# FIT-2023-SLAM-indoor/slam-indoor-code

Hardware: AMD Instinct MI355X
Metric: frames/sec (extract+match+BA) @1080p 10k kpts, 1/2/4/8 GPU; final reproj RMSE (higher is better)
Workload: dtype u8/i8 (int8 MFMA distances, f32 SIFT)

## Files before the change

### slam-indoor-code_amd/csrc/api.cpp

```cpp
#include <algorithm>
#include <cstdlib>
#include <chrono>
#include <cfloat>
#include <cmath>
#include <cstring>
#include <vector>

#include "slamhip_internal.h"

namespace slamhip {

hipError_t DevBuf::ensure(size_t n)
{
    if (n <= bytes && p) return hipSuccess;
    if (p) { (void)hipFree(p); p = nullptr; bytes = 0; }
    size_t want = n < 256 ? 256 : n;
    want = (want + 4095) & ~(size_t)4095;
    hipError_t e = hipMalloc(&p, want);
    if (e == hipSuccess) bytes = want;
    return e;
}

void DevBuf::release()
{
// ... 337 lines not shown
{
    int n = 0;
    if (hipGetDeviceCount(&n) != hipSuccess || device < 0 || device >= n) return nullptr;
    if (hipSetDevice(device) != hipSuccess) return nullptr;
    slam_ctx* c = new slam_ctx();
    c->device = device;
    int least = 0, greatest = 0;
    hipError_t e;
    if (priority > 0 && hipDeviceGetStreamPriorityRange(&least, &greatest) == hipSuccess)
        e = hipStreamCreateWithPriority(&c->stream, hipStreamNonBlocking, greatest);
    else
        e = hipStreamCreateWithFlags(&c->stream, hipStreamNonBlocking);
    if (e != hipSuccess) {
        delete c;
        return nullptr;
    }
    hipDeviceProp_t prop;
    if (hipGetDeviceProperties(&prop, device) == hipSuccess && prop.multiProcessorCount > 0)
        c->cu_count = prop.multiProcessorCount;
    init_consts(c);
    return c;
}

void slam_destroy(slam_ctx* c)
{
    if (!c) return;
    (void)hipSetDevice(c->device);
    (void)hipStreamSynchronize(c->stream);
    DevBuf* bufs[] = {&c->gray, &c->scores, &c->masks, &c->band_cnt, &c->band_pref, &c->frame_info, &c->ftmp,
                      &c->grad, &c->orbblur, &c->kps, &c->kp_frame, &c->desc_u8, &c->desc_f32,
                      &c->desc_norm, &c->desc_exp, &c->query_norm, &c->knn_part, &c->match_rec, &c->match_flag,
                      &c->match_cnt, &c->match_out, &c->frames_in, &c->qbuf, &c->tbuf, &c->misc, &c->ba_obs,
                      &c->ba_par, &c->ba_jac, &c->ba_red, &c->ba_S, &c->ba_aux, &c->sd_pyr, &c->sd_cand,
                      &c->sd_kps, &c->sd_kpc, &c->sift_tab, &c->sift_band_buf, &c->sift_cols_buf, &c->sift_cols_park, &c->sift_colw_buf, &c->sift_split, &c->sift_split_cnt, &c->geom, &c->cluster, &c->delaunay};
    for (DevBuf* b : bufs) b->release();
    if (c->h_up) (void)hipHostFree(c->h_up);
    if (c->ev_up) (void)hipEventDestroy(c->ev_up);
    if (c->h_rb) (void)hipHostFree(c->h_rb);
    if (c->h_win) (void)hipHostFree(c->h_win);
    if (c->ev_win) (void)hipEventDestroy(c->ev_win);
    if (c->ev_rdev) (void)hipEventDestroy(c->ev_rdev);
    if (c->ev_order) (void)hipEventDestroy(c->ev_order);
    for (hipEvent_t e : c->ev_stage)
        if (e) (void)hipEventDestroy(e);
    if (c->h_async) (void)hipHostFree(c->h_async);
    for (auto& f : c->prof)
        for (hipEvent_t e : f.ev) (void)hipEventDestroy(e);
    if (c->ev_sync) (void)hipEventDestroy(c->ev_sync);
    (void)hipStreamDestroy(c->stream);
    delete c;
}

const char* slam_last_error(const slam_ctx* c) { return c ? c->err.c_str() : "no context"; }

int slam_synchronize(slam_ctx* c)
{
    if (!c) return SLAM_E_INVALID_ARG;
    return stream_sync(c, c->stream);
}

int slam_matcher_type(int use_sift_bf, int use_sift_flann, int use_orb)
{
    if (use_sift_bf) return SLAM_SIFT_BF;
    if (use_sift_flann) return SLAM_SIFT_FLANN;
    if (use_orb) return SLAM_ORB_BF;
    return SLAM_E_BAD_MATCHER;
}
// ... 1025 lines not shown
```

### slam-indoor-code_amd/csrc/fast.hip

```cpp
#include "slamhip_internal.h"

namespace slamhip {

namespace {

constexpr int TW = kFastTileW, TH = 4 * kFastTileH;
constexpr int HALO = 4;
constexpr int LW = TW + 2 * HALO;
constexpr int LH = TH + 2 * HALO;
constexpr int SW = TW + 2, SH = TH + 2;
constexpr int SWP = LW;
constexpr int NG = SWP / 4;
static_assert(NG * 4 >= SW + 2, "the last group of a row is past the score columns");
constexpr int kBandsPerTile = TH / kFastTileH;
constexpr int kFastThreads = 256, kFastWaves = kFastThreads / 64;
static_assert(TH % kFastTileH == 0 && kFastWaves % kBandsPerTile == 0 && TH % kFastWaves == 0,
              "whole bands per tile, whole waves per band");
static_assert(TH * 16 % kFastThreads == 0, "whole gray store passes");

struct DetectParams {
    const uint8_t* img;
    size_t frame_stride, row_stride;
    int channels, w, h, thr, border;
    int ntx, nbands;
// ... 322 lines not shown
            int mx = max(max(sc[r][c], sc[r][c + 1]), sc[r][c + 2]);
            mx = max(mx, max(sc[r + 1][c], sc[r + 1][c + 2]));
            mx = max(mx, max(max(sc[r + 2][c], sc[r + 2][c + 1]), sc[r + 2][c + 2]));
            keep = s > mx;
        }
        const int gx = tx * TW + c;
        keep = keep && gx < p.w;
        const bool keepf = keep && gx >= bx && gx < p.w - bx && gy >= bx && gy < p.h - bx;
        kraw |= (uint32_t)keep << (c - 16 * qd);
        kfil |= (uint32_t)keepf << (c - 16 * qd);
        if (keepf) p.scores[(size_t)f * p.w * p.h + (size_t)gy * p.w + gx] = (uint8_t)s;
    }
    uint32_t lo32 = qd == 0 ? kfil : (qd == 1 ? kfil << 16 : 0u);
    uint32_t hi32 = qd == 2 ? kfil : (qd == 3 ? kfil << 16 : 0u);
    lo32 |= __shfl_xor(lo32, 1, 64);
    hi32 |= __shfl_xor(hi32, 1, 64);
    lo32 |= __shfl_xor(lo32, 2, 64);
    hi32 |= __shfl_xor(hi32, 2, 64);
    if (qd == 0 && gy < p.h) p.masks[((size_t)f * p.h + gy) * p.ntx + tx] = ((uint64_t)hi32 << 32) | lo32;
    int craw = __popc(kraw), cfil = __popc(kfil);
#pragma unroll
    for (int o = 32; o > 0; o >>= 1) {
        craw += __shfl_xor(craw, o, 64);
        cfil += __shfl_xor(cfil, o, 64);
    }
    const int band = ty * kBandsPerTile + (tid >> 6);
    if (lane == 0 && band < p.nbands) {
        int* bc = p.band_cnt + ((size_t)f * p.nbands + band) * 2;
        if (craw) atomicAdd(&bc[0], craw);
        if (cfil) atomicAdd(&bc[1], cfil);
    }
}

__global__ __launch_bounds__(1024) void fast_finalize(const int* band_cnt, int nframes, int nbands,
                                                      int* band_pref, int4* frame_info, int* total, int cap)
{
    __shared__ int cnt[1024];
    __shared__ int raw[1024];
    const int lane = threadIdx.x & 63, wave = threadIdx.x >> 6;
    for (int base = 0; base < nframes; base += 1024) {
        for (int fl = wave; fl < 1024 && base + fl < nframes; fl += 16) {
            const int f = base + fl;
            int run = 0, rsum = 0;
            for (int b0 = 0; b0 < nbands; b0 += 64) {
                const int b = b0 + lane;
                int c = 0, r = 0;
                if (b < nbands) {
                    c = band_cnt[((size_t)f * nbands + b) * 2 + 1];
                    r = band_cnt[((size_t)f * nbands + b) * 2 + 0];
                }
                int incl = c;
#pragma unroll
                for (int o = 1; o < 64; o <<= 1) {
                    const int v = __shfl_up(incl, o, 64);
                    if (lane >= o) incl += v;
                }
                if (b < nbands) band_pref[(size_t)f * nbands + b] = run + incl - c;
                run += __shfl(incl, 63, 64);
#pragma unroll
                for (int o = 32; o > 0; o >>= 1) r += __shfl_xor(r, o, 64);
                rsum += r;
            }
            if (lane == 0) { cnt[fl] = run; raw[fl] = rsum; }
        }
        __syncthreads();
        if (threadIdx.x == 0) {
            int off = base == 0 ? 0 : *total;
            for (int i = 0; i < 1024 && base + i < nframes; i++) {
                frame_info[base + i] = make_int4(off, min(cnt[i], max(cap - off, 0)), raw[i], 0);
                off += cnt[i];
            }
            *total = off;
        }
        __syncthreads();
// ... 106 lines not shown
    static const int dbg = [] { return diag_env_int("SLAMHIP_FAST_DBG"); }();
    p.dbg = dbg;
    p.gray = c->gray.as<uint8_t>(); p.masks = c->masks.as<uint64_t>(); p.scores = c->scores.as<uint8_t>();
    p.band_cnt = c->band_cnt.as<int>();
    c->batch.ntx = ntx;
    c->batch.nbands = nbands;
    dim3 grid(ntx, nty, nframes);
    prof_begin(c, 0, s);
    if (type == SLAM_FAST_TYPE_9_16) {
        if (nonmax) hipLaunchKernelGGL((fast_detect<1, 16>), grid, dim3(kFastThreads), 0, s, p);
        else hipLaunchKernelGGL((fast_detect<0, 16>), grid, dim3(kFastThreads), 0, s, p);
    } else if (type == SLAM_FAST_TYPE_7_12) {
        if (nonmax) hipLaunchKernelGGL((fast_detect<1, 12>), grid, dim3(kFastThreads), 0, s, p);
        else hipLaunchKernelGGL((fast_detect<0, 12>), grid, dim3(kFastThreads), 0, s, p);
    } else {
        if (nonmax) hipLaunchKernelGGL((fast_detect<1, 8>), grid, dim3(kFastThreads), 0, s, p);
        else hipLaunchKernelGGL((fast_detect<0, 8>), grid, dim3(kFastThreads), 0, s, p);
    }
    prof_end(c, 0, s);
    return hipGetLastError();
}

hipError_t launch_fast_emit(slam_ctx* c, hipStream_t s, int nframes, int w, int h, int cap)
{
    const int ntx = c->batch.ntx, nbands = c->batch.nbands;
    if (ntx * kFastTileH > 1024) return hipErrorInvalidValue;
    c->fast_gen++;
    hipError_t e;
    if ((e = c->band_pref.ensure((size_t)nframes * nbands * sizeof(int))) != hipSuccess) return e;
    if ((e = c->frame_info.ensure((size_t)nframes * sizeof(int4))) != hipSuccess) return e;
    if ((e = c->misc.ensure(256)) != hipSuccess) return e;
    if ((e = c->kps.ensure((size_t)cap * sizeof(slam_keypoint))) != hipSuccess) return e;
    if ((e = c->kp_frame.ensure((size_t)cap * sizeof(int))) != hipSuccess) return e;
    hipLaunchKernelGGL(fast_finalize, dim3(1), dim3(1024), 0, s, c->band_cnt.as<int>(), nframes, nbands,
                       c->band_pref.as<int>(), c->frame_info.as<int4>(), c->misc.as<int>(), cap);
    EmitParams p;
    p.masks = c->masks.as<uint64_t>(); p.scores = c->scores.as<uint8_t>();
    p.band_pref = c->band_pref.as<int>(); p.frame_info = c->frame_info.as<int4>();
    p.w = w; p.h = h; p.ntx = ntx; p.nbands = nbands; p.cap = cap;
    p.kps = c->kps.as<slam_keypoint>(); p.kp_frame = c->kp_frame.as<int>();
    hipLaunchKernelGGL(fast_emit, dim3(nbands, nframes), dim3(1024), 0, s, p);
    return hipGetLastError();
}

}
```

### slam-indoor-code_amd/csrc/knn.hip

```cpp
#include <cfloat>
#include <climits>
#include <cstdlib>

#include <type_traits>

#include "slamhip_internal.h"

namespace slamhip {

namespace {

typedef int v4i __attribute__((ext_vector_type(4)));
typedef int v16i __attribute__((ext_vector_type(16)));
typedef int v8i __attribute__((ext_vector_type(8)));
typedef float v16f __attribute__((ext_vector_type(16)));

enum { MODE_L2 = 0, MODE_HAM = 1, MODE_SQRT = 2, MODE_L2P = 3, MODE_HAMP = 4, MODE_L1P = 5 };

struct KnnParams {
    const uint8_t* q;
    const int* qnorm;
    int nq;
    const uint8_t* t;
    const int* tnorm;
// ... 686 lines not shown
        if (p.mode == MODE_L2) {
            const int qn = p.qnorm[q];
            if (x0 >= 0) d0 = cr_sqrtf((float)(qn + e0));
            if (x1 >= 0) d1 = cr_sqrtf((float)(qn + e1));
        } else if (p.mode == MODE_HAM) {
            if (x0 >= 0) d0 = (float)((256 + e0) / 2);
            if (x1 >= 0) d1 = (float)((256 + e1) / 2);
        } else if (p.mode == MODE_L2P) {
            const int qn = p.qnorm[q];
            if (x0 >= 0) d0 = cr_sqrtf((float)(qn + e0 - (1 << 21)));
            if (x1 >= 0) d1 = cr_sqrtf((float)(qn + e1 - (1 << 21)));
        } else if (p.mode == MODE_HAMP) {
            if (x0 >= 0) d0 = (float)(e0 / 2);
            if (x1 >= 0) d1 = (float)(e1 / 2);
        } else if (p.mode == MODE_L1P) {
            if (x0 >= 0) d0 = (float)e0;
            if (x1 >= 0) d1 = (float)e1;
        } else {
            if (x0 >= 0) d0 = __int_as_float(e0);
            if (x1 >= 0) d1 = __int_as_float(e1);
        }
        const size_t o = (size_t)fr * p.nq + q;
        if (p.top_idx) { p.top_idx[o] = make_int2(x0, x1); p.top_dist[o] = make_float2(d0, d1); }
        ok = x0 >= 0 && x1 >= 0 && (double)d0 < p.ratio * (double)d1;
        slam_dmatch m;
        m.queryIdx = q; m.trainIdx = x0; m.imgIdx = 0; m.distance = d0;
        p.rec[o] = m;
        p.flag[o] = ok ? 1 : 0;
    }
    const uint64_t b = __ballot(ok);
    if ((threadIdx.x & 63) == 0 && b) atomicAdd(&p.counts[fr], __popcll(b));
}

__global__ __launch_bounds__(1024) void knn_compact(const slam_dmatch* rec, const uint8_t* flag, int nq,
                                                    slam_dmatch* out, int* out_counts, int stride)
{
    __shared__ int wtot[16];
    __shared__ int running;
    const int fr = blockIdx.x, t = threadIdx.x, lane = t & 63, wave = t >> 6;
    if (t == 0) running = 0;
    __syncthreads();
    for (int base = 0; base < nq; base += 1024) {
        const int q = base + t;
        const int f = (q < nq) ? flag[(size_t)fr * nq + q] : 0;
        const uint64_t b = __ballot(f != 0);
        const int below = __popcll(b & ((1ull << lane) - 1));
        if (lane == 0) wtot[wave] = __popcll(b);
        __syncthreads();
        int wb = running;
        for (int i = 0; i < wave; i++) wb += wtot[i];
        if (f) out[(size_t)fr * stride + wb + below] = rec[(size_t)fr * nq + q];
        __syncthreads();
        if (t == 0) { int s = 0; for (int i = 0; i < 16; i++) s += wtot[i]; running += s; }
        __syncthreads();
    }
    if (t == 0) out_counts[fr] = running;
}

int knn_pipe_mode()
{
    static const int m = [] {
        const char* e = getenv("SLAMHIP_KNN_PIPE");
        return e ? atoi(e) : 0;
    }();
    return m;
}
bool knn_pipe_enabled() { return knn_pipe_mode() == 1; }

}

hipError_t launch_knn(slam_ctx* c, hipStream_t s, int kb, const void* q, const int32_t* qnorm, int nq,
                      const void* t, const int32_t* tnorm, const int32_t* t_info, int nframes, int max_nt,
                      int mode, int tsplit, int4* part)
{
    if (nq <= 0 || nframes <= 0) return hipSuccess;
    if (mode == MODE_L2P && (max_nt + tsplit - 1) / tsplit > 1024) return hipErrorInvalidValue;
    if (mode == MODE_HAMP && (max_nt + tsplit - 1) / tsplit > 1024) return hipErrorInvalidValue;
    if (mode == MODE_L1P && (max_nt + tsplit - 1) / tsplit > (1 << 17)) return hipErrorInvalidValue;
    KnnParams p;
    p.q = (const uint8_t*)q; p.qnorm = qnorm; p.nq = nq; p.t = (const uint8_t*)t; p.tnorm = tnorm;
    p.t_info = (const int4*)t_info; p.tsplit = tsplit; p.part = part;
    p.keymul = mode == MODE_HAMP ? -(1 << 22) : -(1 << 11);
    static const int kxcd = [] { const char* e = getenv("SLAMHIP_KNN_XCD"); return e && e[0] == '1' ? 1 : 0; }();
    p.xcd = kxcd;
    const bool pipe1 = kb == 128 && mode == MODE_L2P && knn_pipe_mode() == 2;
    const bool qt1 = kb == 128 && mode == MODE_L2P && knn_pipe_mode() == 3;
// ... 10 lines not shown
        hipLaunchKernelGGL((knn_pipe<KNN_QT, KNN_PIPE_MINB, false>), grid, dim3(256), 0, s, p);
    else if (kb == kOrbExpBytes && mode == MODE_HAMP && knn_pipe_enabled())
        hipLaunchKernelGGL((knn_pipe<2, KNN_PIPE_MINB, true>), grid, dim3(256), 0, s, p);
    else if (kb == 128 && mode == MODE_L2P)
        hipLaunchKernelGGL((knn_mfma_pk<128, false, KNN_QT, KNN_MINB, KNN_NTH>), grid, dim3(KNN_NTH), 0, s, p);
    else if (kb == kOrbExpBytes && mode == MODE_HAMP) hipLaunchKernelGGL((knn_mfma_pk<kOrbExpBytes, true, 2, 4>), grid, dim3(256), 0, s, p);
    else if (kb == 128 && mode == MODE_L1P)
        hipLaunchKernelGGL((knn_l1<2>), dim3((nq + 511) / 512, nframes, tsplit), dim3(256), 0, s, p);
    else { prof_end(c, 2, s); return hipErrorInvalidValue; }
    prof_end(c, 2, s);
    return hipGetLastError();
}

hipError_t launch_knn_finish(slam_ctx* c, hipStream_t s, const int4* part, int nq, int nframes, int tsplit,
                             const int32_t* qnorm, int mode, double ratio, const int32_t* t_info, int2* top_idx,
                             float2* top_dist, slam_dmatch* rec, uint8_t* flag, int32_t* counts)
{
    if (nq <= 0 || nframes <= 0) return hipSuccess;
    FinishParams p;
    p.part = part; p.nq = nq; p.nframes = nframes; p.tsplit = tsplit; p.mode = mode; p.qnorm = qnorm;
    p.ratio = ratio; p.t_info = (const int4*)t_info; p.top_idx = top_idx; p.top_dist = top_dist;
    p.rec = rec; p.flag = flag; p.counts = counts;
    prof_begin(c, 5, s);
    hipLaunchKernelGGL(knn_finish, dim3((nq + 255) / 256, nframes), dim3(256), 0, s, p);
    prof_end(c, 5, s);
    return hipGetLastError();
}

hipError_t launch_compact(slam_ctx* c, hipStream_t s, const slam_dmatch* rec, const uint8_t* flag, int nq,
                          int nframes, slam_dmatch* out, int32_t* out_counts, int stride)
{
    (void)c;
    if (nq <= 0 || nframes <= 0) return hipSuccess;
    hipLaunchKernelGGL(knn_compact, dim3(nframes), dim3(1024), 0, s, rec, flag, nq, out, out_counts, stride);
    return hipGetLastError();
}

}
```

### slam-indoor-code_amd/csrc/sift.hip

```cpp
#include <cfloat>

#include "sift_dev.h"
#include "slamhip_internal.h"

namespace slamhip {

namespace {
using namespace sd;

#ifndef BLUR_DIAG
#define BLUR_DIAG 0
#endif
constexpr int kBT = 64;
constexpr int kBH = 7;
constexpr int kGR = kBT + 2 * kBH;
constexpr int kGL = 80;
#ifndef SIFT_BLUR_GS
#define SIFT_BLUR_GS 96
#endif
constexpr int kGS = SIFT_BLUR_GS;
constexpr int kTW = 68;
constexpr int kTR = kBT + 2;
constexpr int kStrip = 6;
constexpr int kBlurThreads = 512;
// ... 80 lines not shown
    const bf2 a180 = k180 - a;
    a.x = dx.x < 0 ? a180.x : a.x;
    a.y = dx.y < 0 ? a180.y : a.y;
    const bf2 a360 = k360 - a;
    a.x = dy.x < 0 ? a360.x : a.x;
    a.y = dy.y < 0 ? a360.y : a.y;
    const bf2 m2 = __builtin_elementwise_fma(dx, dx, dy * dy);
    const bool tiny = (m2.x > 0.f && m2.x < 0x1p-96f) || (m2.y > 0.f && m2.y < 0x1p-96f);
    if (__builtin_amdgcn_ballot_w64(tiny) == 0)
        return make_float4(sqrt_cr_grad_big(m2.x), a.x, sqrt_cr_grad_big(m2.y), a.y);
    return make_float4(sqrt_cr_grad(m2.x), a.x, sqrt_cr_grad(m2.y), a.y);
}

template <int kOb>
__global__ __launch_bounds__(kBlurThreads) void sift_blur_grad(BlurGradParams p)
{
    constexpr int kGB = kTR * kTW * 4 > kGR * kGS ? kTR * kTW * 4 : kGR * kGS;
    __shared__ __attribute__((aligned(16))) float t[kGR * kTW];
    __shared__ __attribute__((aligned(16))) uint8_t gb_mem[kGB];
    uint8_t* const g = gb_mem;
    float* const b = reinterpret_cast<float*>(gb_mem);
    int bx, by, f;
    xcd_tile(p.xcd != 0, bx, by, f);
    const int x0 = (bx + p.tile0 - 1) * kBT, y0 = (by + p.tile0 - 1) * kBT;
    const int tid = threadIdx.x;
    float2* G = p.grad + (size_t)f * grad_frame(p.w, p.h) + grad_origin(p.w);
    const int pitch = grad_pitch(p.w);
    const float bpr = 8 / 360.f;
    auto stored = [&](float ori) { return kOb ? __fmul_rn(__fsub_rn(ori, p.ori_deg), bpr) : ori; };
    uint8_t* const PB = p.posb + (size_t)f * grad_frame(p.w, p.h) + grad_origin(p.w);
    auto pos_byte = [](float ob) {
        int o0;
        __asm__("v_cvt_flr_i32_f32 %0, %1" : "=v"(o0) : "v"(ob));
        return (uint32_t)((o0 + 9) * 6);
    };
    if (x0 + kBT <= 0 || y0 + kBT <= 0 || x0 >= p.w || y0 >= p.h) {
        const float o0 = stored(0.f);
        const float ov = kOb == 2 ? __builtin_amdgcn_fractf(o0) : o0;
        const uint8_t pb = kOb == 2 ? (uint8_t)pos_byte(o0) : 0;
        for (int i = tid; i < kBT * kBT; i += kBlurThreads) {
            const int x = x0 + (i & 63), y = y0 + (i >> 6);
            if (x >= -kGradPad && x < p.w + kGradPad && y >= -kGradPad && y < p.h + kGradPad) {
                G[(ptrdiff_t)y * pitch + x] = make_float2(0.f, ov);
                if (kOb == 2) PB[(ptrdiff_t)y * pitch + x] = pb;
            }
        }
        return;
    }
    const uint8_t* src = p.gray + (size_t)f * p.w * p.h;

    const bool wide = (p.w & 3) == 0 && x0 - 8 >= 0 && x0 + 72 <= p.w && y0 - kBH >= 0 && y0 + kBT + kBH <= p.h;
    if (wide) {
        for (int i = tid; i < kGR * (kGL / 16); i += kBlurThreads) {
            const int r = i / (kGL / 16), q = i - r * (kGL / 16);
            const uint4 v = *reinterpret_cast<const uint4*>(src + (size_t)(y0 - kBH + r) * p.w + (x0 - 8 + 16 * q));
            *reinterpret_cast<uint4*>(&g[r * kGS + 16 * q]) = v;
        }
    } else {
        for (int i = tid; i < kGR * kGL; i += kBlurThreads) {
            const int r = i / kGL, c = i - r * kGL;
            const int Y = reflect101(y0 - kBH + r, p.h), X = reflect101(x0 - 8 + c, p.w);
            g[r * kGS + c] = src[(size_t)Y * p.w + X];
        }
    }
    __syncthreads();
    bf2 kk[13];
#pragma unroll
// ... 326 lines not shown
```

### slam-indoor-code_amd/csrc/sift_band.hip

```cpp
#include <algorithm>
#include <cfloat>
#include <cmath>
#include <cstdlib>
#include <cstring>
#include <type_traits>
#include <vector>

#include "slamhip_internal.h"

namespace slamhip {

namespace {

#ifndef SIFT_BAND_DIAG_TAB
#define SIFT_BAND_DIAG_TAB 0
#endif
#ifndef SIFT_BAND_DIAG_KP
#define SIFT_BAND_DIAG_KP 0
#endif
#ifndef SIFT_BAND_KS
#define SIFT_BAND_KS 16
#endif
#ifndef SIFT_BAND_WAVES
#define SIFT_BAND_WAVES 8
#endif
#ifndef SIFT_BAND_SLOTCOLS
#define SIFT_BAND_SLOTCOLS 6
#endif
constexpr int kKS = SIFT_BAND_KS;
constexpr int kStride = 2 * kKS + 4;
constexpr int kWaves = SIFT_BAND_WAVES;
constexpr int kKpW = 32;
constexpr int kPos = 10;
constexpr int kCols = 5;
constexpr int kPosF = SIFT_BAND_SLOTCOLS * 64;
static_assert(SIFT_BAND_SLOTCOLS == kCols + 1, "slot columns: the junk column has its own slots");
constexpr int kPos1F = kPosF;
constexpr int kSlots = kPos * kPosF;
constexpr int kStageOff = kSlots;
constexpr int kKpOff = kStageOff + kKpW * kStride;
constexpr int kWaveFloats = kKpOff + kKpW;
constexpr int kMaxChunks = 1024;
constexpr int kTabCols = 5;
constexpr int kRawStride = 129;
static_assert(kKpW * kRawStride <= kKpOff, "epilogue raw buffer must fit below the keypoint offsets");
static_assert(kWaves * kWaveFloats * 4 <= 160 * 1024, "LDS");
static_assert(kStageOff % 4 == 0 && kStride % 4 == 0 && kWaveFloats % 4 == 0, "16-byte stage rows");

namespace q4 {
constexpr int kKpW = 16;
constexpr int kColF = 2 * kKpW;
constexpr int kPosF = 6 * kColF;
constexpr int kCol1F = kKpW;
constexpr int kPos1F = 6 * kCol1F;
constexpr int kSlots = kPos * kPosF;
constexpr int kStageOff = kSlots;
constexpr int kKpOff = kStageOff + kKpW * kStride;
constexpr int kWaveFloats = kKpOff + kKpW;
constexpr int kWaves = 8;
static_assert(kKpW * kRawStride <= kKpOff, "epilogue raw buffer must fit below the keypoint offsets");
static_assert(2 * kWaves * kWaveFloats * 4 <= 160 * 1024, "LDS: two workgroups per CU");
static_assert(kStageOff % 4 == 0 && kWaveFloats % 4 == 0, "16-byte stage rows");
}

struct BandParams {
    const char* grad;
    size_t frame_bytes, origin_bytes;
    int pitch_bytes;
    const slam_keypoint* kps;
    const int* kp_frame;
    const int* total;
    int cap;
    const float2* smp;
    const int* smp_s;
    int nchunks;
    int band_first[6];
    float ori_deg;
    const uint8_t* posb;
    uint8_t* desc_u8;
    float* desc_f32;
    int* norm_i8;
    int wave_major;
    int split;
    int parts_env;
    float4* split_raw;
    int* split_cnt;
};

typedef float f2v __attribute__((ext_vector_type(2)));
typedef int i16v __attribute__((ext_vector_type(16)));
typedef int i8v __attribute__((ext_vector_type(8)));

__device__ __forceinline__ void wave_sync()
{
    __builtin_amdgcn_wave_barrier();
    __asm__ volatile("" ::: "memory");
}

#ifndef SIFT_BAND_ATOMIC
#define SIFT_BAND_ATOMIC 0
#endif
__device__ __forceinline__ void lds_add(float* t, float v)
{
    __hip_atomic_fetch_add(t, v, __ATOMIC_RELAXED, __HIP_MEMORY_SCOPE_WORKGROUP);
}

template <bool kNeg, int kObin>
__global__ __launch_bounds__(64 * kWaves) void sift_desc_band(BandParams p)
{
    __shared__ __attribute__((aligned(16))) float s_buf[kWaves][kWaveFloats];

    const int wave = threadIdx.x >> 6, lane = threadIdx.x & 63;
    const int kq = lane & 31, dc = lane >> 5;
#ifdef SIFT_BAND_PRIO
    if (wave >= 4) __builtin_amdgcn_s_setprio(1);
#endif
    float* buf = s_buf[wave];
    float* stg = buf + kStageOff;
    unsigned* kpo = reinterpret_cast<unsigned*>(buf + kKpOff);
    const float bins_per_rad = 8 / 360.f;
    const float ori_deg = p.ori_deg;

    int total = *p.total;
    if (total > p.cap) total = p.cap;
    const int ngroups = (total + kKpW - 1) / kKpW;
    const int xg = blockIdx.x & 7;
    const int nw = (gridDim.x >> 3) * kWaves;
    const int wi = p.wave_major ? wave * (gridDim.x >> 3) + (blockIdx.x >> 3) : (blockIdx.x >> 3) * kWaves + wave;
    const int per = (ngroups + 7) >> 3;
    const int grp_end = min(ngroups, (xg + 1) * per);
    const int g0 = xg * per, gx = max(0, grp_end - g0);
    const int ncu = (int)(gridDim.x >> 3);
    const bool split_all = p.split >= SLAM_BAND_SPLIT_ALL;
    const int full = split_all ? 0 : gx / nw * nw, rem = gx - full;
    const bool split = rem > 0 && (split_all || (p.split && rem <= ncu));
    const int lg_parts = !split ? 0
                         : split_all ? (p.split == SLAM_BAND_SPLIT_ALL4 ? 2 : 1)
                         : p.parts_env ? (p.parts_env == 4 ? 2 : 1)
                         : (2 * rem > ncu ? 1 : 2);
    const int njobs = split ? full + (rem << lg_parts) : gx;
    const int nch = p.nchunks;
    constexpr int kPairs = kKS / 2, kPer = 64 / kPairs, kIt = kKpW / kPer;
    const int s2 = lane % kPairs, kl = lane / kPairs;
    char* lb = reinterpret_cast<char*>(buf + 2 * kq + dc * 64);
    char* lb1 = reinterpret_cast<char*>(buf + kq + dc * 32);
    char* lb2 = lb - 9 * kPosF * 4;
    char* lb12 = lb1 - 9 * kPos1F * 4;
    const f2v km2 = {dc ? 1.f : 0.f, dc ? 1.f : 0.f}, kn2 = {dc ? -1.f : 1.f, dc ? -1.f : 1.f};
    for (int job = wi; job < njobs; job += nw) {
        int grp = g0 + job, r_lo = 0, r_hi = 3, part = -1;
        if (split && job >= full) {
            grp = g0 + full + ((job - full) >> lg_parts);
            part = (job - full) & ((1 << lg_parts) - 1);
            r_lo = part << (2 - lg_parts);
            r_hi = r_lo + (4 >> lg_parts) - 1;
        }
        const int slot = split_all ? grp : xg * ncu + ((job - full) >> lg_parts);
        const int g = grp * kKpW + kq;
        const bool act = g < total;
        if (dc == 0) {
            const int gg = min(g, total - 1);
            const slam_keypoint kp = p.kps[gg];
            const int ptx = __float2int_rn(kp.x), pty = __float2int_rn(kp.y);
#if SIFT_BAND_DIAG_KP
            (void)ptx; (void)pty;
            kpo[kq] = (unsigned)p.origin_bytes + (unsigned)(500 * p.pitch_bytes + 500 * 8);
#else
            kpo[kq] = (unsigned)((size_t)p.kp_frame[gg] * p.frame_bytes + p.origin_bytes) +
                      (unsigned)(pty * p.pitch_bytes + ptx * 8);
#endif
        }
#pragma unroll 10
        for (int q = 0; q < kSlots / 64; q++) buf[q * 64 + lane] = 0.f;
        wave_sync();
        unsigned kof[kIt];
#pragma unroll
        for (int it = 0; it < kIt; it++) kof[it] = kpo[kPer * it + kl];

        struct Pre { float2 v[2 * kIt]; float wa, wb; uint32_t pb[kIt]; };
        const float4* smp4 = reinterpret_cast<const float4*>(p.smp);
        const int ch0 = p.band_first[r_lo];
        float4 smn = smp4[ch0 * kPairs + s2];
        auto issue = [&](int ch, Pre& pf) __attribute__((always_inline)) {
            const float4 sm = smn;
            pf.wa = sm.x;
            pf.wb = sm.z;
            const unsigned soa = (unsigned)__float_as_int(sm.y), sob = (unsigned)__float_as_int(sm.w);
#pragma unroll
            for (int it = 0; it < kIt; it++) {
                pf.v[2 * it] = *reinterpret_cast<const float2*>(p.grad + (kof[it] + soa));
                pf.v[2 * it + 1] = *reinterpret_cast<const float2*>(p.grad + (kof[it] + sob));
                if constexpr (kObin == 2)
                    pf.pb[it] = *reinterpret_cast<const uint16_t*>(p.posb + ((kof[it] + soa) >> 3));
            }
            smn = smp4[min(ch + 1, nch - 1) * kPairs + s2];
        };
        auto stage = [&](const Pre& pf) __attribute__((always_inline)) {
#pragma unroll
            for (int it = 0; it < kIt; it++) {
                const float2 a = pf.v[2 * it], b = pf.v[2 * it + 1];
                const float mwa = __fmul_rn(a.x, pf.wa), mwb = __fmul_rn(b.x, pf.wb);
                const float oba = kObin ? a.y : __fmul_rn(__fsub_rn(a.y, ori_deg), bins_per_rad);
                const float obb = kObin ? b.y : __fmul_rn(__fsub_rn(b.y, ori_deg), bins_per_rad);
                if constexpr (kObin == 3) {
                    int oa, ob2;
                    __asm__("v_cvt_flr_i32_f32 %0, %1" : "=v"(oa) : "v"(oba));
                    __asm__("v_cvt_flr_i32_f32 %0, %1" : "=v"(ob2) : "v"(obb));
                    *reinterpret_cast<float4*>(stg + (kPer * it + kl) * kStride + 4 * s2) =
                        make_float4(mwa, mwb, __builtin_amdgcn_fractf(oba), __builtin_amdgcn_fractf(obb));
                    *reinterpret_cast<uint16_t*>(reinterpret_cast<char*>(stg + (kPer * it + kl) * kStride + 2 * kKS) + 2 * s2) =
                        (uint16_t)(__mul24(oa + 9, 6) | __mul24(ob2 + 9, 6) << 8);
                    continue;
                }
                if constexpr (kObin < 2) {
                    float* row = stg + (kPer * it + kl) * kStride + 4 * s2;
                    *reinterpret_cast<float2*>(row) = make_float2(mwa, oba);
                    *reinterpret_cast<float2*>(row + 2) = make_float2(mwb, obb);
                    continue;
                }
                *reinterpret_cast<float4*>(stg + (kPer * it + kl) * kStride + 4 * s2) = make_float4(mwa, mwb, oba, obb);
                if constexpr (kObin == 2)
                    *reinterpret_cast<uint16_t*>(reinterpret_cast<char*>(stg + (kPer * it + kl) * kStride + 2 * kKS) + 2 * s2) =
                        (uint16_t)pf.pb[it];
            }
        };

        float raw[4][2][8];
#if SIFT_BAND_KS == 16
        typedef i16v tabv;
#define SIFT_BAND_TABLE_LOAD(trf, tcf, tof, sp)                 \
        __asm__ volatile(                                       \
            "s_load_dwordx16 %0, %3, 0x0\n\t"                   \
            "s_load_dwordx16 %1, %3, 0x40\n\t"                  \
            "s_load_dwordx16 %2, %3, 0x80\n\t"                  \
            "s_waitcnt lgkmcnt(0)"                              \
            : "=&s"(trf), "=&s"(tcf), "=&s"(tof)                \
            : "s"(sp))
#else
        static_assert(kKS == 8, "chunk size");
        typedef i8v tabv;
#define SIFT_BAND_TABLE_LOAD(trf, tcf, tof, sp)                 \
        __asm__ volatile(                                       \
            "s_load_dwordx8 %0, %3, 0x0\n\t"                    \
            "s_load_dwordx8 %1, %3, 0x20\n\t"                   \
// ... 138 lines not shown
#endif
            wave_sync();
        };
#undef SIFT_BAND_TABLE_LOAD
        auto take_row = [&](float (&f)[2][8], const float* c0p, int ps, int cs, int cstride) __attribute__((always_inline)) {
#pragma unroll
            for (int k2 = 0; k2 < 2; k2++) {
                const float* c = c0p + (4 - (2 * dc + k2)) * cstride;
                f[k2][0] = __fadd_rn(c[1 * ps], c[9 * ps]);
                f[k2][1] = __fadd_rn(c[2 * ps], c[-cs]);
#pragma unroll
                for (int q = 2; q < 8; q++) f[k2][q] = c[(q + 1) * ps];
            }
        };
        auto close_band = [&](auto B) __attribute__((always_inline)) {
            constexpr int b = decltype(B)::value;
            if constexpr (b == -1) {
                float v[3][kPos];
#pragma unroll
                for (int c = 0; c < 3; c++)
#pragma unroll
                    for (int ps = 0; ps < kPos; ps++) v[c][ps] = buf[ps * kPos1F + (3 * dc + c) * 32 + kq];
                wave_sync();
#pragma unroll
                for (int c = 0; c < 3; c++)
#pragma unroll
                    for (int ps = 0; ps < kPos; ps++)
                        *reinterpret_cast<float2*>(buf + ps * kPosF + (3 * dc + c) * 64 + 2 * kq) = make_float2(v[c][ps], 0.f);
            } else if constexpr (b <= 2) {
                take_row(raw[b], buf + 2 * kq, kPosF, 64, 64);
                wave_sync();
                if constexpr (b < 2) {
                    float2* z = reinterpret_cast<float2*>(buf);
#pragma unroll 6
                    for (int q = 0; q < kSlots / 128; q++) {
                        float2 vv = z[q * 64 + lane];
                        z[q * 64 + lane] = make_float2(vv.y, 0.f);
                    }
                } else {
                    float v[3][kPos];
#pragma unroll
                    for (int c = 0; c < 3; c++)
#pragma unroll
                        for (int ps = 0; ps < kPos; ps++)
                            v[c][ps] = reinterpret_cast<const float2*>(buf + ps * kPosF + (3 * dc + c) * 64 + 2 * kq)->y;
                    wave_sync();
#pragma unroll
                    for (int c = 0; c < 3; c++)
#pragma unroll
                        for (int ps = 0; ps < kPos; ps++) buf[ps * kPos1F + (3 * dc + c) * 32 + kq] = v[c][ps];
                }
            } else {
                take_row(raw[3], buf + kq, kPos1F, 32, 32);
            }
            wave_sync();
        };

        Pre pf;
        issue(ch0, pf);
        stage(pf);
        wave_sync();
        auto run_band = [&](auto B) __attribute__((always_inline)) {
            constexpr int b = decltype(B)::value;
            const bool skip = b < r_lo - 1 || b > r_hi;
            const int e1 = p.band_first[b + 1], e2 = p.band_first[b + 2];
            const int ch_end = __builtin_amdgcn_readfirstlane(skip ? e1 : e2);
            for (int ch = p.band_first[b + 1]; ch < ch_end; ch++) {
                if (ch + 1 < nch) issue(ch + 1, pf);
// ... 682 lines not shown
    if ((e = c->desc_norm.ensure((size_t)cap * 4)) != hipSuccess) return e;
    if (write_f32 && (e = c->desc_f32.ensure((size_t)cap * 128 * 4)) != hipSuccess) return e;
    const SiftBandMeta& m = c->sift_band;
    BandParams p;
    bool split_ok = false;
    static const int env_split = [] {
        const char* e = getenv("SLAMHIP_SIFT_BAND_SPLIT");
        return e && e[0] >= '0' && e[0] <= '3' ? e[0] - '0' : -1;
    }();
    const int band_split = env_split >= 0 ? env_split : c->opt_band_split;
    p.grad = c->grad.as<char>();
    p.frame_bytes = grad_frame(w, h) * 8;
    p.origin_bytes = grad_origin(w) * 8;
    p.pitch_bytes = grad_pitch(w) * 8;
    p.kps = c->kps.as<slam_keypoint>(); p.kp_frame = c->kp_frame.as<int>(); p.total = c->misc.as<int>();
    p.cap = cap;
    p.smp = c->sift_band_buf.as<float2>();
    p.smp_s = reinterpret_cast<const int*>(c->sift_band_buf.as<char>() + (size_t)m.nrec * sizeof(float2));
    p.nchunks = m.nchunks;
    for (int q = 0; q < 6; q++) p.band_first[q] = m.band_first[q];
    p.ori_deg = m.ori_deg;
    p.posb = c->gradpos.as<uint8_t>();
    if (obin == 2 && (sift_band4_enabled() || !p.posb)) return hipErrorInvalidValue;
    p.desc_u8 = c->desc_u8.as<uint8_t>(); p.desc_f32 = write_f32 ? c->desc_f32.as<float>() : nullptr;
    p.norm_i8 = c->desc_norm.as<int>();
    {
        static const int wm = [] { const char* e = getenv("SLAMHIP_SIFT_BAND_ORDER"); return e && e[0] == '0' ? 0 : 1; }();
        static const int pe = [] { const char* e = getenv("SLAMHIP_SIFT_BAND_PARTS"); return e ? atoi(e) : 0; }();
        p.wave_major = wm;
        p.parts_env = pe == 2 || pe == 4 ? pe : 0;
        p.split = 0;
        p.split_raw = nullptr;
        p.split_cnt = nullptr;
        split_ok = wm && band_split != SLAM_BAND_SPLIT_OFF;
    }
    const bool b4 = sift_band4_enabled();
    int grid = b4 ? 2 * c->cu_count : c->cu_count;
    const int kpb = b4 ? q4::kKpW * q4::kWaves : kKpW * kWaves;
    const int need = (cap + kpb - 1) / kpb;
    if (grid > need) grid = need;
    grid = (grid + 7) & ~7;
    if (grid < 8) grid = 8;
    if (split_ok && !b4) {
        const size_t slots = band_split >= SLAM_BAND_SPLIT_ALL ? (size_t)(cap + kKpW - 1) / kKpW + 8 : (size_t)grid;
        if ((e = c->sift_split.ensure(slots * 4 * 64 * 4 * sizeof(float4))) != hipSuccess) return e;
        const size_t before = c->sift_split_cnt.bytes;
        if ((e = c->sift_split_cnt.ensure(slots * sizeof(int))) != hipSuccess) return e;
        if (c->sift_split_cnt.bytes != before &&
            (e = hipMemsetAsync(c->sift_split_cnt.p, 0, c->sift_split_cnt.bytes, s)) != hipSuccess)
            return e;
        p.split = band_split;
        p.split_raw = c->sift_split.as<float4>();
        p.split_cnt = c->sift_split_cnt.as<int>();
    }
    prof_begin(c, 1, s);
    if (!b4 && obin == 1 && m.neg && c->sift_colw_valid &&
        ((c->opt_sift_kernel == SLAM_SIFT_KERNEL_AUTO && sift_colw_enabled()) ||
         c->opt_sift_kernel == SLAM_SIFT_KERNEL_COLW)) {
        e = launch_sift_desc_colw(c, s, w, h, cap, write_f32);
        prof_end(c, 1, s);
        return e;
    }
    if (!b4 && obin == 1 && m.neg && c->sift_cols_valid &&
        (sift_cols_enabled() || c->opt_sift_kernel == SLAM_SIFT_KERNEL_COLS)) {
        e = launch_sift_desc_cols(c, s, w, h, cap, write_f32);
        prof_end(c, 1, s);
        return e;
    }
    if (b4 && sift_band4_dma()) {
        if (m.neg && obin)
            hipLaunchKernelGGL((sift_desc_band4<true, true, true>), dim3(grid), dim3(64 * q4::kWaves), 0, s, p);
        else if (m.neg)
            hipLaunchKernelGGL((sift_desc_band4<true, false, true>), dim3(grid), dim3(64 * q4::kWaves), 0, s, p);
        else if (obin)
            hipLaunchKernelGGL((sift_desc_band4<false, true, true>), dim3(grid), dim3(64 * q4::kWaves), 0, s, p);
        else
            hipLaunchKernelGGL((sift_desc_band4<false, false, true>), dim3(grid), dim3(64 * q4::kWaves), 0, s, p);
    } else if (b4) {
        if (m.neg && obin)
            hipLaunchKernelGGL((sift_desc_band4<true, true, false>), dim3(grid), dim3(64 * q4::kWaves), 0, s, p);
        else if (m.neg)
            hipLaunchKernelGGL((sift_desc_band4<true, false, false>), dim3(grid), dim3(64 * q4::kWaves), 0, s, p);
        else if (obin)
            hipLaunchKernelGGL((sift_desc_band4<false, true, false>), dim3(grid), dim3(64 * q4::kWaves), 0, s, p);
        else
            hipLaunchKernelGGL((sift_desc_band4<false, false, false>), dim3(grid), dim3(64 * q4::kWaves), 0, s, p);
// ... 20 lines not shown
```

### slam-indoor-code_amd/csrc/slamhip_internal.h

```cpp
#pragma once

#include <hip/hip_runtime.h>

#include <cstddef>
#include <cstdint>
#include <cstdio>
#include <cstdlib>
#include <functional>
#include <utility>
#include <string>
#include <vector>

#include "../../include/slamhip.h"

namespace slamhip {

__device__ __forceinline__ float cr_sqrtf(float x) { return (float)sqrt((double)x); }
__device__ __forceinline__ float cr_divf(float a, float b) { return (float)((double)a / (double)b); }

constexpr int kSiftD = 4, kSiftN = 8;
constexpr int kSiftHist = (kSiftD + 2) * (kSiftD + 2) * (kSiftN + 2);
constexpr int kSiftDescBytes = 128;
constexpr int kOrbDescBytes = 32;
constexpr int kOrbExpBytes = 128;
constexpr int kOrbEdge = 31;

constexpr int kFastTileW = 64, kFastTileH = 16;

struct SiftConsts {
    float gauss[16];
    int ksize;
    float exptab[64];
};

constexpr int kGradPad = 48;
__host__ __device__ __forceinline__ int grad_pitch(int w) { return (w + 2 * kGradPad + 7) & ~7; }

inline bool xcd_tiles_on()
{
    static const bool on = [] { const char* e = getenv("SLAMHIP_XCD_TILES"); return e && e[0] == '1'; }();
    return on;
}
inline int diag_env_int(const char* name)
{
    const char* e = getenv(name);
    if (!e || !e[0]) return 0;
#ifdef SLAMHIP_DIAG
    return atoi(e);
#else
    fprintf(stderr, "slamhip: %s ignored (result-breaking timing probe; build with -DSLAMHIP_DIAG)\n", name);
    return 0;
#endif
}
#ifdef __HIPCC__
__device__ __forceinline__ void xcd_tile(bool on, int& x, int& y, int& z)
{
    x = blockIdx.x; y = blockIdx.y; z = blockIdx.z;
    if (!on) return;
    const unsigned gx = gridDim.x, gy = gridDim.y, n = gx * gy * gridDim.z;
    const unsigned lin = blockIdx.x + gx * (blockIdx.y + gy * blockIdx.z);
    const unsigned per = n >> 3;
    if (lin >= (per << 3)) return;
    const unsigned v = (lin & 7) * per + (lin >> 3);
    x = (int)(v % gx);
    y = (int)((v / gx) % gy);
    z = (int)(v / (gx * gy));
}
#endif
__host__ __device__ __forceinline__ size_t grad_frame(int w, int h)
// ... 103 lines not shown
    size_t h_up_bytes = 0;
    hipEvent_t ev_up = nullptr;
    void* h_win = nullptr;
    size_t h_win_bytes = 0;
    hipEvent_t ev_win = nullptr;
    hipEvent_t ev_rdev = nullptr;
    slamhip::DevBuf synth_world, synth_cams;
    int synth_w = 0, synth_h = 0;
    uint64_t synth_seed = 0;
    int win_pending = 0, win_nk = 0;
    size_t win_kb = 0;
    slamhip::DevBuf frames_in, qbuf, tbuf, misc;
    slamhip::BatchState batch;

    slamhip::DevBuf ba_obs, ba_par, ba_jac, ba_red, ba_S, ba_aux;

    slamhip::DevBuf sd_pyr, sd_cand, sd_kps, sd_kpc;
    slamhip::DevBuf geom;
    slamhip::DevBuf cluster;
    unsigned long long cluster_pairs_total = 0;
    hipStream_t cluster_stats_stream = nullptr;
    slamhip::DevBuf delaunay;
    bool delaunay_ran = false;
    hipStream_t delaunay_stats_stream = nullptr;

    slamhip::DevBuf sift_tab;
    bool sift_tab_valid = false;
    float sift_tab_angle = 0.f, sift_tab_size = 0.f;
    int sift_tab_nrec = 0;
    slamhip::SiftTabMeta sift_meta;
    slamhip::DevBuf sift_band_buf;
    slamhip::DevBuf sift_split;
    slamhip::DevBuf sift_split_cnt;
    bool sift_band_valid = false;
    float sift_band_angle = 0.f, sift_band_size = 0.f;
    slamhip::SiftBandMeta sift_band;
    slamhip::DevBuf sift_cols_buf;
    slamhip::DevBuf sift_cols_park;
    bool sift_cols_valid = false;
    slamhip::SiftColsMeta sift_cols;
    slamhip::DevBuf sift_colw_buf;
    bool sift_colw_valid = false;
    slamhip::SiftColwMeta sift_colw;

    bool prof_on = false;
    slamhip::ProfFamily prof[8];
    int opt_sift_kernel = SLAM_SIFT_KERNEL_AUTO;
    int opt_band_split = SLAM_BAND_SPLIT_AUTO;
    int opt_pnp_sums = SLAM_PNP_SUMS_ORDERED;
    int opt_fast_reuse = 0;
    uint64_t fast_gen = 0;
    struct FastReuse {
        const void* frames = nullptr;
        int nframes = 0, w = 0, h = 0, thr = -1, border = -1, cap = 0;
        uint64_t gen = ~0ull;
    } fast_reuse;
    bool fast_reused = false;
    int last_sift_kernel = 0;
    hipEvent_t ev_order = nullptr;
    hipEvent_t ev_stage[2] = {nullptr, nullptr};
    bool stage_recorded = false;
    struct Async {
        int state = 0;
        hipStream_t s = nullptr;
        int nframes = 0, w = 0, h = 0, matcher = 0, cap = 0;
        bool committed = false;
// ... 114 lines not shown
```

Before: 13400.

## Shrink finalize/compact blocks, compress SIFT band slot layout, add dynamic job dealing

Reduces fast_finalize and knn_compact from 1024 to 256 threads per block. Changes the SIFT band histogram slot layout from 6 to 5 columns per position, with the junk column aliasing discarded slots plus a small pad, which shrinks LDS per wave and the zeroing loop. Adds an atomic work-dealing counter so band-descriptor waves pull full jobs dynamically instead of using a static stride, at the cost of an extra memset and atomics per launch. The layout change risks correctness if the aliasing assumption is wrong.

```diff
diff --git a/slam-indoor-code_amd/csrc/api.cpp b/slam-indoor-code_amd/csrc/api.cpp
--- a/slam-indoor-code_amd/csrc/api.cpp
+++ b/slam-indoor-code_amd/csrc/api.cpp
@@ -393,7 +393,7 @@
                       &c->desc_norm, &c->desc_exp, &c->query_norm, &c->knn_part, &c->match_rec, &c->match_flag,
                       &c->match_cnt, &c->match_out, &c->frames_in, &c->qbuf, &c->tbuf, &c->misc, &c->ba_obs,
                       &c->ba_par, &c->ba_jac, &c->ba_red, &c->ba_S, &c->ba_aux, &c->sd_pyr, &c->sd_cand,
-                      &c->sd_kps, &c->sd_kpc, &c->sift_tab, &c->sift_band_buf, &c->sift_cols_buf, &c->sift_cols_park, &c->sift_colw_buf, &c->sift_split, &c->sift_split_cnt, &c->geom, &c->cluster, &c->delaunay};
+                      &c->sd_kps, &c->sd_kpc, &c->sift_tab, &c->sift_band_buf, &c->sift_cols_buf, &c->sift_cols_park, &c->sift_colw_buf, &c->sift_split, &c->sift_split_cnt, &c->sift_deal, &c->geom, &c->cluster, &c->delaunay};
     for (DevBuf* b : bufs) b->release();
     if (c->h_up) (void)hipHostFree(c->h_up);
     if (c->ev_up) (void)hipEventDestroy(c->ev_up);
diff --git a/slam-indoor-code_amd/csrc/fast.hip b/slam-indoor-code_amd/csrc/fast.hip
--- a/slam-indoor-code_amd/csrc/fast.hip
+++ b/slam-indoor-code_amd/csrc/fast.hip
@@ -378,14 +378,15 @@
     }
 }
 
-__global__ __launch_bounds__(1024) void fast_finalize(const int* band_cnt, int nframes, int nbands,
-                                                      int* band_pref, int4* frame_info, int* total, int cap)
+constexpr int kFinalizeThreads = 256;
+__global__ __launch_bounds__(kFinalizeThreads) void fast_finalize(const int* band_cnt, int nframes, int nbands,
+                                                                  int* band_pref, int4* frame_info, int* total, int cap)
 {
     __shared__ int cnt[1024];
     __shared__ int raw[1024];
     const int lane = threadIdx.x & 63, wave = threadIdx.x >> 6;
     for (int base = 0; base < nframes; base += 1024) {
-        for (int fl = wave; fl < 1024 && base + fl < nframes; fl += 16) {
+        for (int fl = wave; fl < 1024 && base + fl < nframes; fl += kFinalizeThreads / 64) {
             const int f = base + fl;
             int run = 0, rsum = 0;
             for (int b0 = 0; b0 < nbands; b0 += 64) {
@@ -558,7 +559,7 @@
     if ((e = c->misc.ensure(256)) != hipSuccess) return e;
     if ((e = c->kps.ensure((size_t)cap * sizeof(slam_keypoint))) != hipSuccess) return e;
     if ((e = c->kp_frame.ensure((size_t)cap * sizeof(int))) != hipSuccess) return e;
-    hipLaunchKernelGGL(fast_finalize, dim3(1), dim3(1024), 0, s, c->band_cnt.as<int>(), nframes, nbands,
+    hipLaunchKernelGGL(fast_finalize, dim3(1), dim3(kFinalizeThreads), 0, s, c->band_cnt.as<int>(), nframes, nbands,
                        c->band_pref.as<int>(), c->frame_info.as<int4>(), c->misc.as<int>(), cap);
     EmitParams p;
     p.masks = c->masks.as<uint64_t>(); p.scores = c->scores.as<uint8_t>();
diff --git a/slam-indoor-code_amd/csrc/knn.hip b/slam-indoor-code_amd/csrc/knn.hip
--- a/slam-indoor-code_amd/csrc/knn.hip
+++ b/slam-indoor-code_amd/csrc/knn.hip
@@ -742,15 +742,16 @@
     if ((threadIdx.x & 63) == 0 && b) atomicAdd(&p.counts[fr], __popcll(b));
 }
 
-__global__ __launch_bounds__(1024) void knn_compact(const slam_dmatch* rec, const uint8_t* flag, int nq,
-                                                    slam_dmatch* out, int* out_counts, int stride)
-{
-    __shared__ int wtot[16];
+constexpr int kCompactThreads = 256;
+__global__ __launch_bounds__(kCompactThreads) void knn_compact(const slam_dmatch* rec, const uint8_t* flag, int nq,
+                                                               slam_dmatch* out, int* out_counts, int stride)
+{
+    __shared__ int wtot[kCompactThreads / 64];
     __shared__ int running;
     const int fr = blockIdx.x, t = threadIdx.x, lane = t & 63, wave = t >> 6;
     if (t == 0) running = 0;
     __syncthreads();
-    for (int base = 0; base < nq; base += 1024) {
+    for (int base = 0; base < nq; base += kCompactThreads) {
         const int q = base + t;
         const int f = (q < nq) ? flag[(size_t)fr * nq + q] : 0;
         const uint64_t b = __ballot(f != 0);
@@ -761,7 +762,7 @@
         for (int i = 0; i < wave; i++) wb += wtot[i];
         if (f) out[(size_t)fr * stride + wb + below] = rec[(size_t)fr * nq + q];
         __syncthreads();
-        if (t == 0) { int s = 0; for (int i = 0; i < 16; i++) s += wtot[i]; running += s; }
+        if (t == 0) { int s = 0; for (int i = 0; i < kCompactThreads / 64; i++) s += wtot[i]; running += s; }
         __syncthreads();
     }
     if (t == 0) out_counts[fr] = running;
@@ -838,7 +839,7 @@
 {
     (void)c;
     if (nq <= 0 || nframes <= 0) return hipSuccess;
-    hipLaunchKernelGGL(knn_compact, dim3(nframes), dim3(1024), 0, s, rec, flag, nq, out, out_counts, stride);
+    hipLaunchKernelGGL(knn_compact, dim3(nframes), dim3(kCompactThreads), 0, s, rec, flag, nq, out, out_counts, stride);
     return hipGetLastError();
 }
 
diff --git a/slam-indoor-code_amd/csrc/sift.hip b/slam-indoor-code_amd/csrc/sift.hip
--- a/slam-indoor-code_amd/csrc/sift.hip
+++ b/slam-indoor-code_amd/csrc/sift.hip
@@ -136,7 +136,7 @@
     auto pos_byte = [](float ob) {
         int o0;
         __asm__("v_cvt_flr_i32_f32 %0, %1" : "=v"(o0) : "v"(ob));
-        return (uint32_t)((o0 + 9) * 6);
+        return (uint32_t)((o0 + 9) * kBandSlotCols);
     };
     if (x0 + kBT <= 0 || y0 + kBT <= 0 || x0 >= p.w || y0 >= p.h) {
         const float o0 = stored(0.f);
diff --git a/slam-indoor-code_amd/csrc/sift_band.hip b/slam-indoor-code_amd/csrc/sift_band.hip
--- a/slam-indoor-code_amd/csrc/sift_band.hip
+++ b/slam-indoor-code_amd/csrc/sift_band.hip
@@ -24,19 +24,18 @@
 #ifndef SIFT_BAND_WAVES
 #define SIFT_BAND_WAVES 8
 #endif
-#ifndef SIFT_BAND_SLOTCOLS
-#define SIFT_BAND_SLOTCOLS 6
-#endif
 constexpr int kKS = SIFT_BAND_KS;
 constexpr int kStride = 2 * kKS + 4;
 constexpr int kWaves = SIFT_BAND_WAVES;
 constexpr int kKpW = 32;
 constexpr int kPos = 10;
 constexpr int kCols = 5;
-constexpr int kPosF = SIFT_BAND_SLOTCOLS * 64;
-static_assert(SIFT_BAND_SLOTCOLS == kCols + 1, "slot columns: the junk column has its own slots");
+constexpr int kPosF = kBandSlotCols * 64;
+static_assert(kBandSlotCols == kCols, "slot columns: the junk column aliases the quirk column's discarded slots");
+constexpr int kJunkPad = 64;
 constexpr int kPos1F = kPosF;
-constexpr int kSlots = kPos * kPosF;
+static_assert(6 * 32 <= kPos1F, "one-row layout: six columns per position");
+constexpr int kSlots = kPos * kPosF + kJunkPad;
 constexpr int kStageOff = kSlots;
 constexpr int kKpOff = kStageOff + kKpW * kStride;
 constexpr int kWaveFloats = kKpOff + kKpW;
@@ -44,7 +43,7 @@
 constexpr int kTabCols = 5;
 constexpr int kRawStride = 129;
 static_assert(kKpW * kRawStride <= kKpOff, "epilogue raw buffer must fit below the keypoint offsets");
-static_assert(kWaves * kWaveFloats * 4 <= 160 * 1024, "LDS");
+static_assert(kWaves * kWaveFloats * 4 <= 160 * 1024 - 19168, "LDS");
 static_assert(kStageOff % 4 == 0 && kStride % 4 == 0 && kWaveFloats % 4 == 0, "16-byte stage rows");
 
 namespace q4 {
@@ -85,6 +84,7 @@
     int parts_env;
     float4* split_raw;
     int* split_cnt;
+    int* deal;
 };
 
 typedef float f2v __attribute__((ext_vector_type(2)));
@@ -147,7 +147,13 @@
     char* lb2 = lb - 9 * kPosF * 4;
     char* lb12 = lb1 - 9 * kPos1F * 4;
     const f2v km2 = {dc ? 1.f : 0.f, dc ? 1.f : 0.f}, kn2 = {dc ? -1.f : 1.f, dc ? -1.f : 1.f};
-    for (int job = wi; job < njobs; job += nw) {
+    auto take = [&]() __attribute__((always_inline)) {
+        int j = lane == 0 ? atomicAdd(p.deal + xg, 1) : 0;
+        j = __builtin_amdgcn_readfirstlane(j);
+        return j < full ? j : full + wi;
+    };
+    const bool dyn = p.deal != nullptr && full > 0;
+    for (int job = dyn ? take() : wi; job < njobs; job = dyn && job < full ? take() : job + nw) {
         int grp = g0 + job, r_lo = 0, r_hi = 3, part = -1;
         if (split && job >= full) {
             grp = g0 + full + ((job - full) >> lg_parts);
@@ -209,7 +215,7 @@
                     *reinterpret_cast<float4*>(stg + (kPer * it + kl) * kStride + 4 * s2) =
                         make_float4(mwa, mwb, __builtin_amdgcn_fractf(oba), __builtin_amdgcn_fractf(obb));
                     *reinterpret_cast<uint16_t*>(reinterpret_cast<char*>(stg + (kPer * it + kl) * kStride + 2 * kKS) + 2 * s2) =
-                        (uint16_t)(__mul24(oa + 9, 6) | __mul24(ob2 + 9, 6) << 8);
+                        (uint16_t)(__mul24(oa + 9, kBandSlotCols) | __mul24(ob2 + 9, kBandSlotCols) << 8);
                     continue;
                 }
                 if constexpr (kObin < 2) {
@@ -414,8 +420,8 @@
                 wave_sync();
                 if constexpr (b < 2) {
                     float2* z = reinterpret_cast<float2*>(buf);
-#pragma unroll 6
-                    for (int q = 0; q < kSlots / 128; q++) {
+#pragma unroll 5
+                    for (int q = 0; q < kPos * kPosF / 128; q++) {
                         float2 vv = z[q * 64 + lane];
                         z[q * 64 + lane] = make_float2(vv.y, 0.f);
                     }
@@ -1164,6 +1170,7 @@
         p.split = 0;
         p.split_raw = nullptr;
         p.split_cnt = nullptr;
+        p.deal = nullptr;
         split_ok = wm && band_split != SLAM_BAND_SPLIT_OFF;
     }
     const bool b4 = sift_band4_enabled();
@@ -1184,6 +1191,11 @@
         p.split = band_split;
         p.split_raw = c->sift_split.as<float4>();
         p.split_cnt = c->sift_split_cnt.as<int>();
+    }
+    if (!b4) {
+        if ((e = c->sift_deal.ensure(8 * sizeof(int))) != hipSuccess) return e;
+        if ((e = hipMemsetAsync(c->sift_deal.p, 0, 8 * sizeof(int), s)) != hipSuccess) return e;
+        p.deal = c->sift_deal.as<int>();
     }
     prof_begin(c, 1, s);
     if (!b4 && obin == 1 && m.neg && c->sift_colw_valid &&
diff --git a/slam-indoor-code_amd/csrc/slamhip_internal.h b/slam-indoor-code_amd/csrc/slamhip_internal.h
--- a/slam-indoor-code_amd/csrc/slamhip_internal.h
+++ b/slam-indoor-code_amd/csrc/slamhip_internal.h
@@ -35,6 +35,7 @@
 
 constexpr int kGradPad = 48;
 __host__ __device__ __forceinline__ int grad_pitch(int w) { return (w + 2 * kGradPad + 7) & ~7; }
+constexpr int kBandSlotCols = 5;
 
 inline bool xcd_tiles_on()
 {
@@ -204,6 +205,7 @@
     slamhip::DevBuf sift_band_buf;
     slamhip::DevBuf sift_split;
     slamhip::DevBuf sift_split_cnt;
+    slamhip::DevBuf sift_deal;
     bool sift_band_valid = false;
     float sift_band_angle = 0.f, sift_band_size = 0.f;
     slamhip::SiftBandMeta sift_band;
```

Result: faster. 14030 (median of 6 runs) (+4.7%).
